# phandasm/waveform

Measured on NVIDIA H100. Metric: spectra/sec fused window+R2C-FFT+mag+smooth N=2048 batch=65536; %HBM roofline, higher is better.
Workload: dtype f32

## Files before the change

### waveform_b200/csrc/wf_engine.cu

```cuda
#include <cuda_runtime.h>

#include <cmath>
#include <cstdarg>
#include <algorithm>
#include <cstdio>
#include <cstdlib>
#include <cstring>
#include <new>
#include <string>
#include <vector>

#include "wf_kernels.cuh"
#include "wf_fast2048.cuh"
#include "wf_anyn.cuh"
#include "wf_wide.hpp"
#include "wf_v3.hpp"
#include "wf_team2048.hpp"
#include "wf_warp2.hpp"
#include "wf_par16384.hpp"
#include "wf_nvtx.hpp"
#include "wf_tables.hpp"
#include "wfstft.h"

using namespace wf;

struct wf_engine {
    Tables tab;
    int device = 0;
    int sm_count = 0;
    cudaStream_t stream = nullptr;
    cudaEvent_t ev0 = nullptr, ev1 = nullptr;
    bool ev_valid = false;
    std::string last_error;
    int64_t launches = 0;
    std::string last_kernel;
    bool hold_implicit = false;
    bool use_par16384 = true;
    bool use_warp2_display = true;
    bool use_warp2 = true;
    bool lazy_hold = true;
    bool split_runs = true;
    bool force_generic = false;
    int fast_maxw = 16;
    int fast_wpc_override = 0;
    bool use_pdl = true;
    int wide_r = 0;

    float *d_window = nullptr, *d_slope = nullptr, *d_rolloff = nullptr;
    float *d_tw = nullptr, *d_tw_post = nullptr;
    float *d_tw1 = nullptr, *d_tw2 = nullptr, *d_tw0 = nullptr;
    int fast_min_streams = 768;
    int team_w = 0;
    bool use_v3 = true;
    float *d_interp_idx = nullptr, *d_interp_w = nullptr, *d_gauss = nullptr;
    int *d_band_widths = nullptr, *d_band_offsets = nullptr;
    float *d_state = nullptr, *d_hold = nullptr;
    unsigned char *d_flags = nullptr;
    float *s_pcm = nullptr, *s_out_db = nullptr, *s_out_points = nullptr, *s_rms = nullptr, *s_peak = nullptr;
    unsigned char *s_skip = nullptr, *s_silent = nullptr;
    float *s_px = nullptr, *s_min = nullptr;
    float *s_gtab = nullptr;
    size_t s_gtab_cap = 0;
    std::vector<float> h_gtab;
    size_t s_px_cap = 0, s_min_cap = 0;
    float *s_scratch = nullptr;
    size_t s_scratch_cap = 0;
    size_t s_pcm_cap = 0, s_out_db_cap = 0, s_out_points_cap = 0, s_rms_cap = 0, s_peak_cap = 0, s_skip_cap = 0,
           s_silent_cap = 0;
    const void *zc_ptrs[9] = {};
    bool zc_ok = false, zc_dev = false, zc_valid = false;
    bool zero_copy = true;
    static constexpr int kMaxChunks = 16;
    cudaStream_t s_h2d = nullptr, s_d2h = nullptr;
    cudaEvent_t chunk_in[kMaxChunks] = {}, chunk_k[kMaxChunks] = {}, ev_fork = nullptr, ev_join = nullptr;
};

namespace {

thread_local std::string g_create_error;

int set_err(wf_engine *e, int code, const char *fmt, ...)
{
    if(e)
    {
        char buf[512];
        va_list ap;
        va_start(ap, fmt);
        vsnprintf(buf, sizeof(buf), fmt, ap);
        va_end(ap);
        e->last_error = buf;
    }
    return code;
}

#define WF_CUDA(e, call)                                                                                              \
    do                                                                                                                \
// ... 214 lines not shown
    stft_anyn_kernel<CC><<<grid, kAnyThreads, smem, st>>>(kp, plan);
    WF_CUDA(e, cudaGetLastError());
    e->launches++;
    e->last_kernel = "stft_anyn_kernel<" + std::to_string(CC) + "> N=" + std::to_string(e->tab.N);
    return WF_OK;
}

static void fast2048_geometry(int n_streams, int sm_count, int max_wpc, int *warps_per_cta, int *grid)
{
    *grid = std::min(n_streams, sm_count);
    const int per_cta = (n_streams + *grid - 1) / *grid;
    *warps_per_cta = std::max(std::min(8, max_wpc), std::min(max_wpc, per_cta));
}

template<int MAXW, bool TSM, bool GATE, bool EXTRA>
int launch_fast2048(wf_engine *e, const KParams &kp, cudaStream_t st)
{
    static thread_local bool configured[64] = {false};
    const int dev = e->device & 63;
    if(!configured[dev])
    {
        WF_CUDA(e, cudaFuncSetAttribute(stft2048_fast_kernel<MAXW, TSM, GATE, EXTRA>,
                                        cudaFuncAttributeMaxDynamicSharedMemorySize, fast::smem_bytes(MAXW)));
        configured[dev] = true;
    }
    int wpc = MAXW, grid = 1;
    fast2048_geometry(kp.n_streams, e->sm_count, MAXW, &wpc, &grid);
    if(e->fast_wpc_override > 0 && e->fast_wpc_override <= MAXW)
    {
        wpc = e->fast_wpc_override;
        grid = std::min(kp.n_streams, e->sm_count);
    }
    cudaLaunchConfig_t cfg{};
    cfg.gridDim = dim3((unsigned)grid);
    cfg.blockDim = dim3((unsigned)(wpc * 32));
    cfg.dynamicSmemBytes = fast::smem_bytes(wpc);
    cfg.stream = st;
    cudaLaunchAttribute attr[1];
    attr[0].id = cudaLaunchAttributeProgrammaticStreamSerialization;
    attr[0].val.programmaticStreamSerializationAllowed = e->use_pdl ? 1 : 0;
    cfg.attrs = attr;
    cfg.numAttrs = 1;
    WF_CUDA(e, cudaLaunchKernelEx(&cfg, stft2048_fast_kernel<MAXW, TSM, GATE, EXTRA>, kp));
    e->launches++;
    e->last_kernel = "stft2048_fast_kernel<" + std::to_string(MAXW) + "," + std::to_string((int)TSM) + "," + std::to_string((int)GATE) +
                     "," + std::to_string((int)EXTRA) + "> grid " + std::to_string(grid) + " x " + std::to_string(wpc) + " warps";
    return WF_OK;
}


int dispatch_fast2048(wf_engine *e, const KParams &kp, cudaStream_t st, bool extra)
{
    const bool tsm = kp.tsmooth != 0, gate = kp.gate != 0;
    const int maxw = e->fast_maxw;
#define WF_FAST_CASE(W, T, G, X)            \
    if(maxw == W && tsm == T && gate == G && extra == X) \
        return launch_fast2048<W, T, G, X>(e, kp, st);
    WF_FAST_CASE(16, true, true, false)
    WF_FAST_CASE(16, true, true, true)
    WF_FAST_CASE(16, true, false, false)
    WF_FAST_CASE(16, true, false, true)
    WF_FAST_CASE(16, false, true, false)
    WF_FAST_CASE(16, false, true, true)
    WF_FAST_CASE(16, false, false, false)
    WF_FAST_CASE(16, false, false, true)
    WF_FAST_CASE(12, true, true, false)
    WF_FAST_CASE(12, true, true, true)
    WF_FAST_CASE(12, true, false, false)
    WF_FAST_CASE(12, true, false, true)
    WF_FAST_CASE(12, false, true, false)
    WF_FAST_CASE(12, false, true, true)
    WF_FAST_CASE(12, false, false, false)
    WF_FAST_CASE(12, false, false, true)
#undef WF_FAST_CASE
    return set_err(e, WF_ERR_INVALID_ARG, "fast2048 dispatch fell through");
}

int fill_device(wf_engine *e, float *p, long long n, float v, cudaStream_t st)
{
    if(n <= 0)
        return WF_OK;
    int blocks = (int)std::min<long long>((n + 255) / 256, 1184);
    fill_kernel<<<blocks, 256, 0, st>>>(p, n, v);
    WF_CUDA(e, cudaGetLastError());
    e->launches++;
    return WF_OK;
}

int materialize_hold(wf_engine *e, cudaStream_t st)
{
    if(!e->hold_implicit)
        return WF_OK;
    const Tables &t = e->tab;
    const int S = t.cfg.max_streams;
    materialize_hold_kernel<<<std::min(S, e->sm_count * 8), 256, 0, st>>>(e->d_state, e->d_hold, e->d_flags, S, t.B,
                                                                          t.output_channels, t.db_min);
    WF_CUDA(e, cudaGetLastError());
    e->launches++;
    e->hold_implicit = false;
    return WF_OK;
}

int init_state(wf_engine *e, int first, int count, cudaStream_t st)
{
    const Tables &t = e->tab;
    const int cc = t.cfg.capture_channels, och = t.output_channels, B = t.B;
    WF_CUDA(e, cudaMemsetAsync(e->d_state + (size_t)first * cc * B, 0, (size_t)count * cc * B * sizeof(float), st));
    int rc = fill_device(e, e->d_hold + (size_t)first * och * B, (long long)count * och * B, t.db_min, st);
    if(rc)
        return rc;
    const bool below = !(t.db_min > (float)(t.cfg.floor_db - 10));
    WF_CUDA(e, cudaMemsetAsync(e->d_flags + first, below ? 6 : 0, (size_t)count, st));
    return WF_OK;
}

}

extern "C" {

int wf_abi_version(void) { return WF_ABI_VERSION; }

const char *wf_strerror(int status)
{
    switch(status)
    {
    case WF_OK: return "ok";
// ... 45 lines not shown
    c->interp_mode = WF_INTERP_CATROM;
    c->filter_mode = WF_FILTER_NONE;
    c->filter_radius = 1.5f;
    c->height = 225;
    c->channel_spacing = 0;
    c->rounded_caps = 0;
    c->min_bar_height = 0;
}

int wf_create(const wf_config *cfg, wf_engine **out)
{
    if(!cfg || !out)
        return WF_ERR_INVALID_ARG;
    *out = nullptr;
    if(cfg->struct_size != sizeof(wf_config))
        return WF_ERR_ABI;
    wf_engine *e = new(std::nothrow) wf_engine();
    if(!e)
        return WF_ERR_OOM;
    auto bail = [&](int code) {
        g_create_error = e->last_error;
        wf_destroy(e);
        return code;
    };

    const char *why = nullptr;
    int rc = build_tables(*cfg, e->tab, &why);
    if(rc != WF_OK)
    {
        set_err(e, rc, "%s", why ? why : "bad config");
        return bail(rc);
    }
    if(!supported_fft_size(e->tab.N))
        return bail(set_err(e, WF_ERR_UNSUPPORTED_FFT_SIZE, "fft_size %d unsupported", e->tab.N));

    int ndev = 0;
    if(cudaGetDeviceCount(&ndev) != cudaSuccess || ndev == 0)
    {
        cudaGetLastError();
        return bail(set_err(e, WF_ERR_NO_DEVICE, "no CUDA device"));
    }
    int dev = cfg->device;
    if(dev < 0)
    {
        if(cudaGetDevice(&dev) != cudaSuccess)
            return bail(set_err(e, WF_ERR_CUDA, "cudaGetDevice failed"));
    }
    if(dev >= ndev)
        return bail(set_err(e, WF_ERR_INVALID_ARG, "device %d out of range (%d devices)", dev, ndev));
    e->device = dev;
    {
        const char *fg = getenv("WF_FORCE_GENERIC");
        e->force_generic = fg && fg[0] == '1';
        const char *mw = getenv("WF_FAST_MAXW");
        if(mw && (atoi(mw) == 12 || atoi(mw) == 16))
            e->fast_maxw = atoi(mw);
        const char *np = getenv("WF_NO_PDL");
        e->use_pdl = !(np && np[0] == '1');
        const char *wr = getenv("WF_WIDE_R");
        if(wr)
            e->wide_r = atoi(wr);
        const char *fms = getenv("WF_FAST_MIN_STREAMS");
        if(fms)
            e->fast_min_streams = atoi(fms);
        const char *v3 = getenv("WF_V3");
        e->use_v3 = !(v3 && v3[0] == '0');
        const char *tw = getenv("WF_TEAM_W");
        if(tw)
            e->team_w = atoi(tw);
        const char *zc = getenv("WF_ZERO_COPY");
        e->zero_copy = !(zc && zc[0] == '0');
        const char *p16 = getenv("WF_PAR16384");
        e->use_par16384 = !(p16 && p16[0] == '0');
        const char *w2 = getenv("WF_WARP2");
        e->use_warp2 = !(w2 && w2[0] == '0');
        const char *w2d = getenv("WF_WARP2_DISPLAY");
        e->use_warp2_display = !(w2d && w2d[0] == '0');
        const char *lh = getenv("WF_LAZY_HOLD");
        e->lazy_hold = !(lh && lh[0] == '0');
        const char *sp = getenv("WF_SPLIT");
        e->split_runs = !(sp && sp[0] == '0');
        const char *wo = getenv("WF_FAST_WPC");
        if(wo)
            e->fast_wpc_override = atoi(wo);
    }

#define WF_TRY(x)                 \
    do                            \
    {                             \
        int _rc = (x);            \
        if(_rc != WF_OK)          \
            return bail(_rc);     \
    } while(0)
#define WF_CUDA_C(call)                                                                                      \
    do                                                                                                       \
    {                                                                                                        \
        cudaError_t _err = (call);                                                                           \
        if(_err != cudaSuccess)                                                                              \
            return bail(set_err(e, (_err == cudaErrorMemoryAllocation) ? WF_ERR_OOM : WF_ERR_CUDA, "%s: %s", \
                                #call, cudaGetErrorString(_err)));                                           \
    } while(0)

    WF_CUDA_C(cudaSetDevice(dev));
    cudaDeviceProp prop{};
    WF_CUDA_C(cudaGetDeviceProperties(&prop, dev));
    e->sm_count = prop.multiProcessorCount;
    if(prop.major != 9 || prop.minor != 0)
        return bail(set_err(e, WF_ERR_NO_DEVICE, "device %d is sm_%d%d; this library is built for sm_90a only", dev,
                            prop.major, prop.minor));
// ... 191 lines not shown
    kp.fast_peaks = t.cfg.fast_peaks;
    kp.stereo = t.cfg.stereo;
    kp.och = och;
    kp.dch = dch;
    kp.gate = t.cfg.silence_gate;
    kp.floor_m10 = (float)(t.cfg.floor_db - 10);
    kp.db_min = t.db_min;
    kp.normalize = t.cfg.normalize_volume;
    kp.vol_target = t.cfg.volume_target;
    kp.max_gain = t.cfg.max_gain;
    kp.write_hold = 1;
    kp.interp_idx = e->d_interp_idx;
    kp.interp_w = e->d_interp_w;
    kp.band_widths = e->d_band_widths;
    kp.band_offsets = e->d_band_offsets;
    kp.n_points = t.num_points;
    kp.n_sample = (t.cfg.display_mode == WF_DISPLAY_BAR && t.cfg.interp_mode != WF_INTERP_POINT) ? (int)t.interp_indices.size() : 0;
    kp.scratch_q = t.num_points + (dch * kp.n_sample + 3) / 4;
    kp.taps = t.interp_taps;
    kp.radius = t.interp_radius;
    kp.display_bar = (t.cfg.display_mode == WF_DISPLAY_BAR);
    kp.interp_mode = t.cfg.interp_mode;
    kp.gauss_w = e->d_gauss;
    kp.gauss_radius = t.gauss_radius;
    kp.gauss_size = (int)t.gauss.size();
    kp.gauss_sum = t.gauss_sum;
    kp.filter = (t.cfg.filter_mode == WF_FILTER_GAUSS);
    kp.out_pixels = b->out_pixels ? px_dev + (size_t)s0 * T * dch * t.num_points : nullptr;
    kp.out_min = b->out_min ? min_dev + (size_t)s0 * T * 2 : nullptr;
    kp.px_lo = t.px_lo;
    kp.px_hi = t.px_hi;
    kp.px_cpos = t.px_cpos;
    kp.ceiling_f = (float)t.cfg.ceiling_db;
    kp.dbrange_f = (float)(t.cfg.ceiling_db - t.cfg.floor_db);
    kp.mirror = t.cfg.mirror_freq_axis;

    size_t extra = 0;
    if(kp.out_points || kp.out_pixels || kp.out_min)
    {
        int groups = 1;
        switch(N)
        {
        case 128: groups = Geo<128>::GROUPS; break;
        case 256: groups = Geo<256>::GROUPS; break;
        case 512: groups = Geo<512>::GROUPS; break;
        case 1024: groups = Geo<1024>::GROUPS; break;
        case 2048: groups = Geo<2048>::GROUPS; break;
        default: groups = 1; break;
        }
        extra = (size_t)groups * 4 * (size_t)kp.scratch_q * sizeof(float);
    }
    const bool aligned16 = (((uintptr_t)kp.pcm & 15u) == 0) && ((b->stream_stride & 3) == 0) && ((b->hop & 3) == 0);
    const bool fast_ok = (N == 2048) && (cc == 1) && !t.cfg.stereo && kp.out_db && !kp.out_points && !kp.out_pixels &&
                         !kp.out_min && aligned16 && !e->force_generic;
    if(fast_ok)
    {
        const bool x = kp.slope || kp.rolloff || kp.normalize || kp.fast_peaks || kp.skip_mask || kp.out_peak || kp.g_tab;
        kp.lazy_hold = e->lazy_hold ? 1 : 0;
        kp.split = e->split_runs ? 1 : 0;
        if(kp.lazy_hold)
            e->hold_implicit = true;
        int W = 1;
        if(e->team_w != 1)
        {
            const int per_sm = (kp.n_streams + e->sm_count - 1) / e->sm_count;
            if(per_sm <= 8)
                W = (per_sm <= 1) ? 16 : (per_sm == 2) ? 8 : 4;
            if(e->team_w == 4 || e->team_w == 8 || e->team_w == 16)
                W = e->team_w;
            while(W > 1 && W > kp.n_frames)
                W /= 2;
            if(W == 2)
                W = 1;
        }
        if(W > 1)
        {
            const int tpc = 16 / W;
            const int grid = std::min(e->sm_count, kp.n_streams);
            WF_CUDA(e, team2048_launch(W, x, kp, grid, st, e->use_pdl, e->device));
            e->launches++;
            e->last_kernel = "stft2048_team_kernel<" + std::to_string(W) + "," + std::to_string((int)x) + "> grid " + std::to_string(grid) +
                             " x " + std::to_string(tpc) + " teams";
            return WF_OK;
        }
        return dispatch_fast2048(e, kp, st, x);
    }
    {
        const int rc = materialize_hold(e, st);
        if(rc)
            return rc;
    }
    const bool par_ok = (N == 16384) && e->use_par16384 && e->use_v3 && e->d_tw0 && (cc == 1) && !t.cfg.stereo && kp.out_db &&
                        !kp.out_points && !kp.out_pixels && !kp.out_min && !e->force_generic;
    if(par_ok)
    {
        const bool x = kp.slope || kp.rolloff || kp.normalize || kp.fast_peaks || kp.skip_mask || kp.out_peak || kp.g_tab;
        WF_CUDA(e, par16384_launch(x, kp, e->d_tw1, e->d_tw2, e->d_tw0, st, e->device));
        e->launches++;
        e->last_kernel = "stft16384_parity_kernel<" + std::to_string((int)x) + "> " + std::to_string(kp.n_streams) + " clusters of 2";
        return WF_OK;
    }
    const bool disp = kp.out_points || kp.out_pixels || kp.out_min;
    const bool warp2_ok = e->use_warp2 && (cc == 1) && !t.cfg.stereo && aligned16 &&
                          (disp ? (e->use_warp2_display && !e->force_generic && (warp2_supported(N) || warp2_pow2_supported(N)))
                                : (warp2_supported(N) && kp.out_db));
    if(warp2_ok)
    {
// ... 444 lines not shown
```

### waveform_b200/csrc/wf_fast2048.cuh

```cuda
#pragma once
#include "wf_kernels.cuh"

namespace wf {

namespace fast {

constexpr int kN = 2048;
constexpr int kM = 1024;
constexpr int kWarpBufBytes = 32 * 33 * 8;
constexpr int kStateBytes = 16 * 32 * 8;
constexpr int kWarpBytes = kWarpBufBytes + kStateBytes + 16;
constexpr int kTableBytes = (1024 + 1024 + 512) * 8;
constexpr int kMaxWarpsPerCta = 16;
constexpr int smem_bytes(int warps_per_cta) { return kTableBytes + warps_per_cta * kWarpBytes; }

__device__ __forceinline__ uint32_t smem_u32(const void *p) { return (uint32_t)__cvta_generic_to_shared(p); }

__device__ __forceinline__ void mbar_init(uint64_t *bar, uint32_t count)
{
    asm volatile("mbarrier.init.shared::cta.b64 [%0], %1;" ::"r"(smem_u32(bar)), "r"(count) : "memory");
}
__device__ __forceinline__ void mbar_expect_tx(uint64_t *bar, uint32_t bytes)
{
    asm volatile("mbarrier.arrive.expect_tx.shared::cta.b64 _, [%0], %1;" ::"r"(smem_u32(bar)), "r"(bytes) : "memory");
}
__device__ __forceinline__ void mbar_wait(uint64_t *bar, uint32_t parity)
{
    asm volatile(
        "{\n\t"
        ".reg .pred p;\n\t"
        "WAIT_LOOP:\n\t"
        "mbarrier.try_wait.parity.shared::cta.b64 p, [%0], %1;\n\t"
        "@p bra DONE;\n\t"
        "bra WAIT_LOOP;\n\t"
        "DONE:\n\t"
        "}" ::"r"(smem_u32(bar)),
        "r"(parity)
        : "memory");
}
__device__ __forceinline__ void tma_load_1d(void *dst_smem, const void *src_gmem, uint32_t bytes, uint64_t *bar)
{
    asm volatile("cp.async.bulk.shared::cluster.global.mbarrier::complete_tx::bytes [%0], [%1], %2, [%3];" ::"r"(
                     smem_u32(dst_smem)),
                 "l"(src_gmem), "r"(bytes), "r"(smem_u32(bar))
                 : "memory");
}
__device__ __forceinline__ void fence_proxy_async()
{
    asm volatile("fence.proxy.async.shared::cta;" ::: "memory");
}
__device__ __forceinline__ float sqrt_approx(float x)
{
    float r;
    asm("sqrt.approx.ftz.f32 %0, %1;" : "=f"(r) : "f"(x));
    return r;
}

__device__ __forceinline__ float lg2_approx_ftz(float x)
{
    float r;
    asm("lg2.approx.ftz.f32 %0, %1;" : "=f"(r) : "f"(x));
    return r;
}
__device__ __forceinline__ pk::c64 dbfs2(float m1, float m2, float db_min)
{
    constexpr float k = 6.02059991327962390f;
    pk::c64 d = pk::mul(pk::make(lg2_approx_ftz(m1), lg2_approx_ftz(m2)), pk::make(k, k));
    float d1, d2;
    pk::split(d, d1, d2);
    return pk::make(fmaxf(d1, db_min), fmaxf(d2, db_min));
}

}

template<int MAXW, bool TSM, bool GATE, bool EXTRA>
__global__ void __launch_bounds__(MAXW * 32, 1) stft2048_fast_kernel(const __grid_constant__ KParams p)
{
    using namespace fast;
    extern __shared__ __align__(128) unsigned char smem_raw[];
    float2 *s_win = reinterpret_cast<float2 *>(smem_raw);
    float2 *s_twA = s_win + 1024;
    float2 *s_twP = s_twA + 1024;
    const int warp = threadIdx.x >> 5;
    const int lane = threadIdx.x & 31;
    const int warps_per_cta = blockDim.x >> 5;
    unsigned char *wbase = reinterpret_cast<unsigned char *>(s_twP + 512) + warp * kWarpBytes;
    float2 *buf = reinterpret_cast<float2 *>(wbase);
    float2 *sst = reinterpret_cast<float2 *>(wbase + kWarpBufBytes) + lane;
    uint64_t *mbar = reinterpret_cast<uint64_t *>(wbase + kWarpBufBytes + kStateBytes);

    for(int i = threadIdx.x; i < 1024; i += blockDim.x)
    {
        {
            const float2 w = (p.window2 != nullptr) ? __ldg(p.window2 + i) : make_float2(1.0f, 1.0f);
            s_win[i] = make_float2(w.x * p.coef_half, w.y * p.coef_half);
        }
        s_twA[i] = __ldg(p.tw + (((i >> 5) * (i & 31)) & 1023));
        if(i < 512)
            s_twP[i] = __ldg(p.tw_post + i);
    }
    int *seg_done = reinterpret_cast<int *>(mbar + 1);
    if(lane == 0)
    {
        mbar_init(mbar, 1);
        *seg_done = 0;
        asm volatile("fence.mbarrier_init.release.cluster;" ::: "memory");
    }
    __syncthreads();
    asm volatile("griddepcontrol.launch_dependents;" ::: "memory");
    asm volatile("griddepcontrol.wait;" ::: "memory");

    const int S = p.n_streams, T = p.n_frames;
    const int G = gridDim.x;
    const int n_local = (S > (int)blockIdx.x) ? (S - (int)blockIdx.x + G - 1) / G : 0;
    constexpr int B = kM;
    uint32_t phase = 0;

    const int jp = (32 - lane) & 31;
    const int kb = jp + (lane == 0 ? 32 : 0);
    const int k2_q0 = (lane == 0) ? 512 : (kb + 992);

    const int rounds_whole = (n_local + warps_per_cta - 1) / warps_per_cta;
    const bool split = (p.split != 0) && (n_local >= warps_per_cta) && (T > 1) &&
                       (2 * (rounds_whole * warps_per_cta - n_local) * T > 3 * warps_per_cta);
    int u0 = 0, u1 = 0;
    if(split)
    {
        const int U = n_local * T, per = (U + warps_per_cta - 1) / warps_per_cta;
        u0 = min(warp * per, U);
        u1 = min(u0 + per, U);
    }
    const int full0 = (u0 + T - 1) / T, full1 = u1 / T;
    const int has_head = (split && (u1 % T) != 0) ? 1 : 0, has_tail = (split && (u0 % T) != 0) ? 1 : 0;
    const int nseg = split ? (has_head + max(full1 - full0, 0) + has_tail)
                           : ((n_local > warp) ? (n_local - warp + warps_per_cta - 1) / warps_per_cta : 0);
    auto segment = [&](int j, int &li, int &t0, int &t1) {
        if(!split)
        {
            li = warp + j * warps_per_cta;
            t0 = 0;
            t1 = T;
            return;
        }
        if(has_head && j == 0)
        {
            li = full1;
            t0 = 0;
            t1 = u1 % T;
            return;
        }
        j -= has_head;
        if(j < full1 - full0)
        {
            li = full0 + j;
            t0 = 0;
            t1 = T;
            return;
        }
        li = u0 / T;
        t0 = u0 % T;
        t1 = T;
    };

    if(nseg > 0 && lane == 0)
    {
        int li, t0, t1;
        segment(0, li, t0, t1);
        mbar_expect_tx(mbar, kN * 4);
        tma_load_1d(buf, p.pcm + (size_t)(blockIdx.x + li * G) * p.stream_stride + (size_t)t0 * p.hop, kN * 4, mbar);
    }

    for(int j = 0; j < nseg; ++j)
    {
        int li, t0, t1;
        segment(j, li, t0, t1);
        const int s = (int)blockIdx.x + li * G;
        int s_next = -1, t0_next = 0;
        if(j + 1 < nseg)
        {
            int li2, t12;
            segment(j + 1, li2, t0_next, t12);
            s_next = (int)blockIdx.x + li2 * G;
        }
        if(t0 > 0)
        {
            int *prev_done = reinterpret_cast<int *>(wbase - kWarpBytes + kWarpBufBytes + kStateBytes + 8);
            if(lane == 0)
                while(atomicAdd(prev_done, 0) == 0)
                    ;
            __syncwarp();
            __threadfence_block();
        }
        {
            const float *sp = p.state + (size_t)s * B;
#pragma unroll
            for(int q = 0; q < 16; ++q)
                sst[q * 32] = make_float2(sp[lane + 32 * q], sp[(q == 0) ? k2_q0 : (kb + 32 * (31 - q))]);
        }
        const unsigned char fl = p.flags[s];
        bool last_silent = (fl & 1u) != 0;
        bool prev_out_silent = (fl & 2u) != 0;
        const bool hold_lazy = (fl & 8u) != 0;
        bool last_from_state = false;
        const float *pcm_s = p.pcm + (size_t)s * p.stream_stride;
        float *hold_s = p.hold_db + (size_t)s * B;

#pragma unroll 1
        for(int t = t0; t < t1; ++t)
        {
            mbar_wait(mbar, phase);
            phase ^= 1u;
            pk::c64 v[32];
            unsigned long long nzbits = 0;
            const pk::c64 *buf64 = reinterpret_cast<const pk::c64 *>(buf);
            const pk::c64 *win64 = reinterpret_cast<const pk::c64 *>(s_win);
#pragma unroll
            for(int pidx = 0; pidx < 32; ++pidx)
            {
                v[pidx] = buf64[lane + 32 * pidx];
                nzbits |= v[pidx];
            }
#pragma unroll
            for(int pidx = 0; pidx < 32; ++pidx)
                v[pidx] = pk::mul(v[pidx], win64[lane + 32 * pidx]);
            const bool nz = __any_sync(0xffffffffu, (nzbits & 0x7fffffff7fffffffull) != 0ull);

#pragma unroll
            for(int pass = 0; pass < 2; ++pass)
            {
                pk::dft_bitrev<32>(v);
                if(pass == 0)
                {
                    __syncwarp();
#pragma unroll
                    for(int k2 = 0; k2 < 32; ++k2)
                    {
                        pk::c64 a = v[bitrev<32>(k2)];
                        if(k2 > 0)
                            a = pk::cmul(a, reinterpret_cast<const pk::c64 *>(s_twA)[k2 * 32 + lane]);
                        reinterpret_cast<pk::c64 *>(buf)[lane * 33 + k2] = a;
                    }
                    __syncwarp();
#pragma unroll
                    for(int n1 = 0; n1 < 32; ++n1)
                        v[n1] = buf64[n1 * 33 + lane];
                    __syncwarp();
                    if(t + 1 == t1 && s_next >= 0 && t0_next == 0)
                        asm volatile("prefetch.global.L2 [%0];" ::"l"(p.state + (size_t)s_next * B + lane * 32));
                    if(lane == 0)
                    {
                        const float *next = nullptr;
                        if(t + 1 < t1)
                            next = pcm_s + (size_t)(t + 1) * p.hop;
                        else if(s_next >= 0)
                            next = p.pcm + (size_t)s_next * p.stream_stride + (size_t)t0_next * p.hop;
                        if(next != nullptr)
                        {
                            fence_proxy_async();
                            mbar_expect_tx(mbar, kN * 4);
                            tma_load_1d(buf, next, kN * 4, mbar);
                        }
                    }
                }
            }

            const bool skip_all = EXTRA && (p.skip_mask != nullptr) && (p.skip_mask[(size_t)s * T + t] != 0);
            bool do_proc = !skip_all;
            if(!skip_all)
            {
                if(nz)
                    last_silent = false;
                else if(GATE)
                {
                    if(last_silent)
                        do_proc = false;
                    else if(prev_out_silent)
                    {
                        last_silent = true;
                        do_proc = false;
                    }
                }
            }

            float *odb = p.out_db + ((size_t)s * T + t) * B;
            float vc = 0.0f;
            if(EXTRA && p.normalize)
            {
                const float rms = (p.input_rms != nullptr) ? p.input_rms[(size_t)s * T + t] : 0.0f;
                vc = fminf(p.vol_target - dbfs(rms, p.db_min), p.max_gain);
            }
            bool outs = true;
            float peak = -INFINITY;
            const float2 gt = (EXTRA && p.g_tab != nullptr) ? __ldg(p.g_tab + t) : make_float2(p.g, p.g2);

            if(do_proc && !last_silent)
            {
#pragma unroll
                for(int q = 0; q < 16; ++q)
                {
                    const int k1 = lane + 32 * q;
                    const int k2 = (q == 0) ? k2_q0 : (kb + 32 * (31 - q));
                    const pk::c64 a = v[bitrev<32>(q)];
                    unsigned long long bp = __shfl_sync(0xffffffffu, v[bitrev<32>(31 - q)], jp);
                    if(lane == 0)
                        bp = v[bitrev<32>((32 - q) & 31)];
                    const pk::c64 b = pk::conj(bp);
                    const pk::c64 sum = pk::add(a, b);
                    const pk::c64 o = pk::mul_neg_i(pk::sub(a, b));
                    const pk::c64 wo = pk::cmul(o, reinterpret_cast<const pk::c64 *>(s_twP)[q * 32 + lane]);
                    const pk::c64 y1 = pk::add(sum, wo);
                    const pk::c64 y2 = pk::sub(sum, wo);
                    const pk::c64 s1 = pk::mul(y1, y1), s2 = pk::mul(y2, y2);
                    float p1 = pk::re(s1) + pk::im(s1);
                    float p2 = pk::re(s2) + pk::im(s2);
                    if(q == 0)
                    {
                        const pk::c64 x512 = v[bitrev<32>(16)];
                        const pk::c64 sq = pk::mul(x512, x512);
                        const float p512 = 4.0f * (pk::re(sq) + pk::im(sq));
                        p2 = (lane == 0) ? p512 : p2;
                    }
                    pk::c64 m = pk::make(sqrt_approx(p1), sqrt_approx(p2));
                    if(EXTRA && p.slope != nullptr)
                        m = pk::mul(m, pk::make(__ldg(p.slope + k1), __ldg(p.slope + k2)));
                    pk::c64 *sst64 = reinterpret_cast<pk::c64 *>(sst);
                    if(TSM)
                    {
                        pk::c64 old = sst64[q * 32];
                        if(EXTRA && p.fast_peaks)
                            old = pk::make(fmaxf(pk::re(m), pk::re(old)), fmaxf(pk::im(m), pk::im(old)));
                        m = pk::fma(pk::make(gt.x, gt.x), old, pk::mul(pk::make(gt.y, gt.y), m));
                    }
                    sst64[q * 32] = m;
                    float d1, d2;
                    pk::split(dbfs2(pk::re(m), pk::im(m), p.db_min), d1, d2);
                    if(EXTRA)
                    {
                        if(p.normalize)
                        {
                            if(k1 >= 1)
                                d1 += vc;
                            d2 += vc;
                        }
                        if(p.rolloff != nullptr)
                        {
                            if(k1 >= 1)
                                d1 = fmaxf(d1 - __ldg(p.rolloff + k1), p.db_min);
                            d2 = fmaxf(d2 - __ldg(p.rolloff + k2), p.db_min);
                        }
                        if(k1 >= 1)
                            peak = fmaxf(peak, d1);
                        peak = fmaxf(peak, d2);
                    }
                    if(GATE)
                        outs &= !(d1 > p.floor_m10) & !(d2 > p.floor_m10);
                    stg_stream(odb + k1, d1);
                    stg_stream(odb + k2, d2);
                }
                last_from_state = true;
            }
            else
            {
                const float *prev_db = (t > 0) ? (odb - B) : hold_s;
                const bool from_state = (t == 0) && hold_lazy;
#pragma unroll 1
                for(int q = 0; q < 16; ++q)
                {
                    const int k1 = lane + 32 * q;
                    const int k2 = (q == 0) ? k2_q0 : (kb + 32 * (31 - q));
                    float o1, o2;
                    if(from_state)
                    {
                        const float2 stv = sst[q * 32];
                        pk::split(dbfs2(stv.x, stv.y, p.db_min), o1, o2);
                    }
                    else
                    {
                        o1 = prev_db[k1];
                        o2 = prev_db[k2];
                    }
                    if(!last_silent)
                    {
                        o1 = dbfs(o1, p.db_min);
                        o2 = dbfs(o2, p.db_min);
                        if(EXTRA)
                        {
                            if(p.normalize)
                            {
                                if(k1 >= 1)
                                    o1 += vc;
                                o2 += vc;
                            }
                            if(p.rolloff != nullptr)
                            {
                                if(k1 >= 1)
                                    o1 = fmaxf(o1 - __ldg(p.rolloff + k1), p.db_min);
                                o2 = fmaxf(o2 - __ldg(p.rolloff + k2), p.db_min);
                            }
                        }
                    }
                    outs &= !(o1 > p.floor_m10) & !(o2 > p.floor_m10);
                    if(k1 >= 1)
                        peak = fmaxf(peak, o1);
                    peak = fmaxf(peak, o2);
                    odb[k1] = o1;
                    odb[k2] = o2;
                }
                last_from_state = false;
            }
            if(GATE && !last_silent)
                prev_out_silent = __all_sync(0xffffffffu, outs);
            if(p.out_silent != nullptr && lane == 0)
                p.out_silent[(size_t)s * T + t] = last_silent ? 1 : 0;
            if(EXTRA)
            {
                if(p.out_peak != nullptr)
                {
                    const float gm = group_max<32>(peak, nullptr);
                    if(lane == 0)
                        atomic_max_float(p.out_peak + t, gm);
                }
            }
        }

        {
            float *sp = p.state + (size_t)s * B;
            const float *last = p.out_db + ((size_t)s * T + (t1 - 1)) * B;
            const bool plain = !EXTRA || (!p.normalize && p.rolloff == nullptr);
            const bool lazy = last_from_state && plain && (p.lazy_hold != 0);
#pragma unroll
            for(int q = 0; q < 16; ++q)
            {
                const int k1 = lane + 32 * q;
                const int k2 = (q == 0) ? k2_q0 : (kb + 32 * (31 - q));
                const float2 stv = sst[q * 32];
                sp[k1] = stv.x;
                sp[k2] = stv.y;
                if(p.write_hold && !lazy)
                {
                    if(last_from_state && plain)
                    {
                        float h1, h2;
                        pk::split(dbfs2(stv.x, stv.y, p.db_min), h1, h2);
                        hold_s[k1] = h1;
                        hold_s[k2] = h2;
                    }
                    else
                    {
                        hold_s[k1] = last[k1];
                        hold_s[k2] = last[k2];
                    }
                }
            }
            if(lane == 0)
                p.flags[s] = (unsigned char)((last_silent ? 1u : 0u) | (prev_out_silent ? 2u : 0u) | 4u | (lazy ? 8u : 0u));
        }
        if(t1 < T)
        {
            __threadfence_block();
            __syncwarp();
            if(lane == 0)
                atomicExch(seg_done, 1);
        }
        __syncwarp();
    }
}

}
```

### waveform_b200/csrc/wf_team2048.cuh

```cuda
#pragma once
#include "wf_fast2048.cuh"

namespace wf {

namespace team {
constexpr int kCtlBytes = 64;
constexpr int kWarps = 16;
constexpr int smem_bytes() { return fast::kTableBytes + kWarps * fast::kWarpBytes + kWarps * kCtlBytes; }

__device__ __forceinline__ void bar_sync(int id, int nthreads)
{
    asm volatile("bar.sync %0, %1;" ::"r"(id), "r"(nthreads) : "memory");
}
}

template<int W, bool EXTRA>
__global__ void __launch_bounds__(team::kWarps * 32, 1) stft2048_team_kernel(const __grid_constant__ KParams p)
{
    using namespace fast;
    constexpr int TPC = team::kWarps / W;
    constexpr int BW = kM / W;
    constexpr int BPL = BW / 32;
    constexpr int VEC = (BPL >= 4) ? 4 : 2;
    constexpr int B = kM;
    extern __shared__ __align__(128) unsigned char smem_raw[];
    float2 *s_win = reinterpret_cast<float2 *>(smem_raw);
    float2 *s_twA = s_win + 1024;
    float2 *s_twP = s_twA + 1024;
    const int warp = threadIdx.x >> 5;
    const int lane = threadIdx.x & 31;
    const int tm = warp / W;
    const int wi = warp % W;
    unsigned char *warps_base = reinterpret_cast<unsigned char *>(s_twP + 512);
    unsigned char *wbase = warps_base + warp * kWarpBytes;
    float2 *buf = reinterpret_cast<float2 *>(wbase);
    float *mymag = reinterpret_cast<float *>(wbase + kWarpBufBytes);
    uint64_t *mbar = reinterpret_cast<uint64_t *>(wbase + kWarpBufBytes + kStateBytes);
    unsigned char *ctl = warps_base + team::kWarps * kWarpBytes + tm * team::kCtlBytes;
    volatile unsigned char *ctl_nz = ctl;
    volatile unsigned char *ctl_outs = ctl + 16;
    const int bar_id = 1 + tm;

    for(int i = threadIdx.x; i < 1024; i += blockDim.x)
    {
        const float2 w = (p.window2 != nullptr) ? __ldg(p.window2 + i) : make_float2(1.0f, 1.0f);
        s_win[i] = make_float2(w.x * p.coef_half, w.y * p.coef_half);
        s_twA[i] = __ldg(p.tw + (((i >> 5) * (i & 31)) & 1023));
        if(i < 512)
            s_twP[i] = __ldg(p.tw_post + i);
    }
    if(lane == 0)
    {
        mbar_init(mbar, 1);
        asm volatile("fence.mbarrier_init.release.cluster;" ::: "memory");
    }
    __syncthreads();
    asm volatile("griddepcontrol.launch_dependents;" ::: "memory");
    asm volatile("griddepcontrol.wait;" ::: "memory");

    const int S = p.n_streams, T = p.n_frames;
    const int G = gridDim.x;
    const int n_local = (S > (int)blockIdx.x) ? (S - (int)blockIdx.x + G - 1) / G : 0;
    uint32_t phase = 0;
    const bool tsm = p.tsmooth != 0, gate = p.gate != 0;

    const int jp = (32 - lane) & 31;
    const int kb = jp + (lane == 0 ? 32 : 0);
    const int k2_q0 = (lane == 0) ? 512 : (kb + 992);
    const int b0 = wi * BW + lane * BPL;

    if(tm < n_local && wi < T && lane == 0)
    {
        mbar_expect_tx(mbar, kN * 4);
        tma_load_1d(buf, p.pcm + (size_t)(blockIdx.x + tm * G) * p.stream_stride + (size_t)wi * p.hop, kN * 4, mbar);
    }

    for(int li = tm; li < n_local; li += TPC)
    {
        const int s = (int)blockIdx.x + li * G;
        const bool have_next_stream = (li + TPC) < n_local;
        const float *pcm_s = p.pcm + (size_t)s * p.stream_stride;
        float *hold_s = p.hold_db + (size_t)s * B;
        float *state_s = p.state + (size_t)s * B;

        float st[BPL];
#pragma unroll
        for(int j = 0; j < BPL; j += VEC)
        {
            if constexpr(VEC == 4)
            {
                const float4 x = *reinterpret_cast<const float4 *>(state_s + b0 + j);
// ... 86 lines not shown
                    const int k1 = lane + 32 * q;
                    const int k2 = (q == 0) ? k2_q0 : (kb + 32 * (31 - q));
                    const pk::c64 a = v[bitrev<32>(q)];
                    unsigned long long bp = __shfl_sync(0xffffffffu, v[bitrev<32>(31 - q)], jp);
                    if(lane == 0)
                        bp = v[bitrev<32>((32 - q) & 31)];
                    const pk::c64 b = pk::conj(bp);
                    const pk::c64 sum = pk::add(a, b);
                    const pk::c64 o = pk::mul_neg_i(pk::sub(a, b));
                    const pk::c64 wo = pk::cmul(o, reinterpret_cast<const pk::c64 *>(s_twP)[q * 32 + lane]);
                    const pk::c64 y1 = pk::add(sum, wo);
                    const pk::c64 y2 = pk::sub(sum, wo);
                    const pk::c64 s1 = pk::mul(y1, y1), s2 = pk::mul(y2, y2);
                    float p1 = pk::re(s1) + pk::im(s1);
                    float p2 = pk::re(s2) + pk::im(s2);
                    if(q == 0)
                    {
                        const pk::c64 x512 = v[bitrev<32>(16)];
                        const pk::c64 sq = pk::mul(x512, x512);
                        const float p512 = 4.0f * (pk::re(sq) + pk::im(sq));
                        p2 = (lane == 0) ? p512 : p2;
                    }
                    float m1 = sqrt_approx(p1), m2 = sqrt_approx(p2);
                    if(EXTRA && p.slope != nullptr)
                    {
                        m1 *= __ldg(p.slope + k1);
                        m2 *= __ldg(p.slope + k2);
                    }
                    mymag[k1] = m1;
                    mymag[k2] = m2;
                }
                if(lane == 0)
                    ctl_nz[wi] = nz ? 1 : 0;
            }
            team::bar_sync(bar_id, W * 32);

            bool round_done = false;
            if(t0 + W <= T && !(EXTRA && p.skip_mask != nullptr))
            {
                bool all_nz = true;
#pragma unroll
                for(int i = 0; i < W; ++i)
                    all_nz &= ctl_nz[i] != 0;
                if(all_nz)
                {
                    last_silent = false;
                    float *odb0 = p.out_db + ((size_t)s * T + t0) * B + b0;
                    float dl[BPL];
#pragma unroll
                    for(int i = 0; i < W; ++i)
                    {
                        const int tt = t0 + i;
                        const float2 gt = (EXTRA && p.g_tab != nullptr) ? __ldg(p.g_tab + tt) : make_float2(p.g, p.g2);
                        const float *mg = reinterpret_cast<const float *>(warps_base + (size_t)(tm * W + i) * kWarpBytes + kWarpBufBytes) + b0;
                        float d[BPL];
#pragma unroll
                        for(int j = 0; j < BPL; j += VEC)
                        {
                            float m[4];
                            if constexpr(VEC == 4)
                            {
                                const float4 x = *reinterpret_cast<const float4 *>(mg + j);
                                m[0] = x.x, m[1] = x.y, m[2] = x.z, m[3] = x.w;
                            }
                            else
                            {
                                const float2 x = *reinterpret_cast<const float2 *>(mg + j);
                                m[0] = x.x, m[1] = x.y;
                            }
#pragma unroll
                            for(int u = 0; u < VEC; ++u)
                            {
                                float mm = m[u];
                                if(tsm)
                                {
                                    float old = st[j + u];
                                    if(EXTRA && p.fast_peaks)
                                        old = fmaxf(mm, old);
                                    mm = fmaf(gt.x, old, gt.y * mm);
                                }
                                st[j + u] = mm;
                            }
                        }
#pragma unroll
                        for(int j = 0; j < BPL; j += 2)
                            pk::split(dbfs2(st[j], st[j + 1], p.db_min), d[j], d[j + 1]);
                        if(EXTRA)
                        {
                            float vc = 0.0f;
                            if(p.normalize)
                            {
                                const float rms = (p.input_rms != nullptr) ? p.input_rms[(size_t)s * T + tt] : 0.0f;
                                vc = fminf(p.vol_target - dbfs(rms, p.db_min), p.max_gain);
                            }
                            float peak = -INFINITY;
#pragma unroll
                            for(int j = 0; j < BPL; ++j)
                            {
                                const int k = b0 + j;
                                if(k >= 1)
                                {
                                    if(p.normalize)
                                        d[j] += vc;
                                    if(p.rolloff != nullptr)
                                        d[j] = fmaxf(d[j] - __ldg(p.rolloff + k), p.db_min);
                                    peak = fmaxf(peak, d[j]);
                                }
// ... 31 lines not shown
                            outs &= !(dl[j] > p.floor_m10);
                        outs_lane = outs;
                        pos_valid = false;
                    }
                    if(p.out_silent != nullptr && wi == 0 && lane < W)
                        p.out_silent[(size_t)s * T + t0 + lane] = 0;
                    last_from_state = true;
                    round_done = true;
                }
            }
#pragma unroll 1
            for(int i = 0; i < W && !round_done; ++i)
            {
                const int tt = t0 + i;
                if(tt >= T)
                    break;
                const bool nz = ctl_nz[i] != 0;
                const bool skip_all = EXTRA && (p.skip_mask != nullptr) && (p.skip_mask[(size_t)s * T + tt] != 0);
                bool do_proc = !skip_all;
                if(!skip_all)
                {
                    if(nz)
                        last_silent = false;
                    else if(gate)
                    {
                        if(last_silent)
                            do_proc = false;
                        else
                        {
                            if(!pos_valid)
                            {
                                pos = team_all(outs_lane);
                                pos_valid = true;
                            }
                            if(pos)
                            {
                                last_silent = true;
                                do_proc = false;
                            }
                        }
                    }
                }
                const float2 gt = (EXTRA && p.g_tab != nullptr) ? __ldg(p.g_tab + tt) : make_float2(p.g, p.g2);
                float *odb = p.out_db + ((size_t)s * T + tt) * B + b0;
                float vc = 0.0f;
                if(EXTRA && p.normalize)
                {
                    const float rms = (p.input_rms != nullptr) ? p.input_rms[(size_t)s * T + tt] : 0.0f;
                    vc = fminf(p.vol_target - dbfs(rms, p.db_min), p.max_gain);
                }
                float d[BPL];
                if(do_proc && !last_silent)
                {
                    const float *mg = reinterpret_cast<const float *>(warps_base + (size_t)(tm * W + i) * kWarpBytes + kWarpBufBytes) + b0;
#pragma unroll
                    for(int j = 0; j < BPL; j += VEC)
                    {
                        float m[4];
                        if constexpr(VEC == 4)
                        {
                            const float4 x = *reinterpret_cast<const float4 *>(mg + j);
                            m[0] = x.x, m[1] = x.y, m[2] = x.z, m[3] = x.w;
                        }
                        else
                        {
                            const float2 x = *reinterpret_cast<const float2 *>(mg + j);
                            m[0] = x.x, m[1] = x.y;
                        }
#pragma unroll
                        for(int u = 0; u < VEC; ++u)
                        {
                            float mm = m[u];
                            if(tsm)
                            {
                                float old = st[j + u];
                                if(EXTRA && p.fast_peaks)
                                    old = fmaxf(mm, old);
                                mm = fmaf(gt.x, old, gt.y * mm);
                            }
                            st[j + u] = mm;
                        }
                    }
#pragma unroll
                    for(int j = 0; j < BPL; j += 2)
                    {
                        pk::split(dbfs2(st[j], st[j + 1], p.db_min), d[j], d[j + 1]);
                    }
                    if(EXTRA)
                    {
#pragma unroll
                        for(int j = 0; j < BPL; ++j)
                        {
                            const int k = b0 + j;
                            if(k >= 1)
                            {
                                if(p.normalize)
                                    d[j] += vc;
                                if(p.rolloff != nullptr)
                                    d[j] = fmaxf(d[j] - __ldg(p.rolloff + k), p.db_min);
                            }
                        }
                    }
                    last_from_state = true;
                }
                else
                {
                    const bool from_state = (tt == 0) && hold_lazy;
// ... 106 lines not shown
```

Measured before the change: 192.9 million.

## Add TMA landing buffer, register smoothing state, and bulk async row stores

Each warp gets a separate landing buffer for the input frame, so the next frame's TMA load can be issued right after the current frame is read instead of after the first FFT pass. Smoothing state moves from shared memory into registers. Output dB rows are staged in shared memory and written with cp.async.bulk stores instead of per-lane streaming stores. The larger per-warp shared footprint lowers the maximum warps per CTA from 16 to 12, which cuts parallelism per SM, and the fast path now also requires a 16-byte-aligned output pointer.

```diff
diff --git a/waveform_b200/csrc/wf_engine.cu b/waveform_b200/csrc/wf_engine.cu
--- a/waveform_b200/csrc/wf_engine.cu
+++ b/waveform_b200/csrc/wf_engine.cu
@@ -41,7 +41,6 @@
     bool lazy_hold = true;
     bool split_runs = true;
     bool force_generic = false;
-    int fast_maxw = 16;
     int fast_wpc_override = 0;
     bool use_pdl = true;
     int wide_r = 0;
@@ -362,26 +361,17 @@
 int dispatch_fast2048(wf_engine *e, const KParams &kp, cudaStream_t st, bool extra)
 {
     const bool tsm = kp.tsmooth != 0, gate = kp.gate != 0;
-    const int maxw = e->fast_maxw;
-#define WF_FAST_CASE(W, T, G, X)            \
-    if(maxw == W && tsm == T && gate == G && extra == X) \
-        return launch_fast2048<W, T, G, X>(e, kp, st);
-    WF_FAST_CASE(16, true, true, false)
-    WF_FAST_CASE(16, true, true, true)
-    WF_FAST_CASE(16, true, false, false)
-    WF_FAST_CASE(16, true, false, true)
-    WF_FAST_CASE(16, false, true, false)
-    WF_FAST_CASE(16, false, true, true)
-    WF_FAST_CASE(16, false, false, false)
-    WF_FAST_CASE(16, false, false, true)
-    WF_FAST_CASE(12, true, true, false)
-    WF_FAST_CASE(12, true, true, true)
-    WF_FAST_CASE(12, true, false, false)
-    WF_FAST_CASE(12, true, false, true)
-    WF_FAST_CASE(12, false, true, false)
-    WF_FAST_CASE(12, false, true, true)
-    WF_FAST_CASE(12, false, false, false)
-    WF_FAST_CASE(12, false, false, true)
+#define WF_FAST_CASE(T, G, X)                  \
+    if(tsm == T && gate == G && extra == X) \
+        return launch_fast2048<fast::kMaxWarpsPerCta, T, G, X>(e, kp, st);
+    WF_FAST_CASE(true, true, false)
+    WF_FAST_CASE(true, true, true)
+    WF_FAST_CASE(true, false, false)
+    WF_FAST_CASE(true, false, true)
+    WF_FAST_CASE(false, true, false)
+    WF_FAST_CASE(false, true, true)
+    WF_FAST_CASE(false, false, false)
+    WF_FAST_CASE(false, false, true)
 #undef WF_FAST_CASE
     return set_err(e, WF_ERR_INVALID_ARG, "fast2048 dispatch fell through");
 }
@@ -533,9 +523,6 @@
     {
         const char *fg = getenv("WF_FORCE_GENERIC");
         e->force_generic = fg && fg[0] == '1';
-        const char *mw = getenv("WF_FAST_MAXW");
-        if(mw && (atoi(mw) == 12 || atoi(mw) == 16))
-            e->fast_maxw = atoi(mw);
         const char *np = getenv("WF_NO_PDL");
         e->use_pdl = !(np && np[0] == '1');
         const char *wr = getenv("WF_WIDE_R");
@@ -833,7 +820,7 @@
     }
     const bool aligned16 = (((uintptr_t)kp.pcm & 15u) == 0) && ((b->stream_stride & 3) == 0) && ((b->hop & 3) == 0);
     const bool fast_ok = (N == 2048) && (cc == 1) && !t.cfg.stereo && kp.out_db && !kp.out_points && !kp.out_pixels &&
-                         !kp.out_min && aligned16 && !e->force_generic;
+                         !kp.out_min && aligned16 && (((uintptr_t)kp.out_db & 15u) == 0) && !e->force_generic;
     if(fast_ok)
     {
         const bool x = kp.slope || kp.rolloff || kp.normalize || kp.fast_peaks || kp.skip_mask || kp.out_peak || kp.g_tab;
diff --git a/waveform_b200/csrc/wf_fast2048.cuh b/waveform_b200/csrc/wf_fast2048.cuh
--- a/waveform_b200/csrc/wf_fast2048.cuh
+++ b/waveform_b200/csrc/wf_fast2048.cuh
@@ -7,12 +7,13 @@
 
 constexpr int kN = 2048;
 constexpr int kM = 1024;
-constexpr int kWarpBufBytes = 32 * 33 * 8;
-constexpr int kStateBytes = 16 * 32 * 8;
-constexpr int kWarpBytes = kWarpBufBytes + kStateBytes + 16;
+constexpr int kLandBytes = kN * 4;
+constexpr int kXposeBytes = 32 * 33 * 8;
+constexpr int kWarpBytes = kLandBytes + kXposeBytes + 16;
 constexpr int kTableBytes = (1024 + 1024 + 512) * 8;
-constexpr int kMaxWarpsPerCta = 16;
+constexpr int kMaxWarpsPerCta = 12;
 constexpr int smem_bytes(int warps_per_cta) { return kTableBytes + warps_per_cta * kWarpBytes; }
+static_assert(smem_bytes(kMaxWarpsPerCta) <= 227 * 1024, "one CTA per SM must fit");
 
 __device__ __forceinline__ uint32_t smem_u32(const void *p) { return (uint32_t)__cvta_generic_to_shared(p); }
 
@@ -49,6 +50,21 @@
 {
     asm volatile("fence.proxy.async.shared::cta;" ::: "memory");
 }
+__device__ __forceinline__ void bulk_store_1d(void *dst_gmem, const void *src_smem, uint32_t bytes)
+{
+    asm volatile("cp.async.bulk.global.shared::cta.bulk_group [%0], [%1], %2;" ::"l"(dst_gmem), "r"(smem_u32(src_smem)), "r"(bytes)
+                 : "memory");
+    asm volatile("cp.async.bulk.commit_group;" ::: "memory");
+}
+__device__ __forceinline__ void bulk_wait_read()
+{
+    asm volatile("cp.async.bulk.wait_group.read 0;" ::: "memory");
+}
+__device__ __forceinline__ void bulk_wait_written()
+{
+    asm volatile("cp.async.bulk.wait_group 0;" ::: "memory");
+    asm volatile("fence.proxy.async.global;" ::: "memory");
+}
 __device__ __forceinline__ float sqrt_approx(float x)
 {
     float r;
@@ -77,6 +93,7 @@
 __global__ void __launch_bounds__(MAXW * 32, 1) stft2048_fast_kernel(const __grid_constant__ KParams p)
 {
     using namespace fast;
+    static_assert(MAXW <= kMaxWarpsPerCta, "shared memory holds at most kMaxWarpsPerCta warps");
     extern __shared__ __align__(128) unsigned char smem_raw[];
     float2 *s_win = reinterpret_cast<float2 *>(smem_raw);
     float2 *s_twA = s_win + 1024;
@@ -85,9 +102,11 @@
     const int lane = threadIdx.x & 31;
     const int warps_per_cta = blockDim.x >> 5;
     unsigned char *wbase = reinterpret_cast<unsigned char *>(s_twP + 512) + warp * kWarpBytes;
-    float2 *buf = reinterpret_cast<float2 *>(wbase);
-    float2 *sst = reinterpret_cast<float2 *>(wbase + kWarpBufBytes) + lane;
-    uint64_t *mbar = reinterpret_cast<uint64_t *>(wbase + kWarpBufBytes + kStateBytes);
+    float2 *land = reinterpret_cast<float2 *>(wbase);
+    float2 *buf = reinterpret_cast<float2 *>(wbase + kLandBytes);
+    float *row = reinterpret_cast<float *>(buf);
+    uint64_t *mbar = reinterpret_cast<uint64_t *>(wbase + kWarpBytes - 16);
+    pk::c64 st[16];
 
     for(int i = threadIdx.x; i < 1024; i += blockDim.x)
     {
@@ -167,7 +186,7 @@
         int li, t0, t1;
         segment(0, li, t0, t1);
         mbar_expect_tx(mbar, kN * 4);
-        tma_load_1d(buf, p.pcm + (size_t)(blockIdx.x + li * G) * p.stream_stride + (size_t)t0 * p.hop, kN * 4, mbar);
+        tma_load_1d(land, p.pcm + (size_t)(blockIdx.x + li * G) * p.stream_stride + (size_t)t0 * p.hop, kN * 4, mbar);
     }
 
     for(int j = 0; j < nseg; ++j)
@@ -184,7 +203,7 @@
         }
         if(t0 > 0)
         {
-            int *prev_done = reinterpret_cast<int *>(wbase - kWarpBytes + kWarpBufBytes + kStateBytes + 8);
+            int *prev_done = reinterpret_cast<int *>(reinterpret_cast<unsigned char *>(seg_done) - kWarpBytes);
             if(lane == 0)
                 while(atomicAdd(prev_done, 0) == 0)
                     ;
@@ -195,7 +214,7 @@
             const float *sp = p.state + (size_t)s * B;
 #pragma unroll
             for(int q = 0; q < 16; ++q)
-                sst[q * 32] = make_float2(sp[lane + 32 * q], sp[(q == 0) ? k2_q0 : (kb + 32 * (31 - q))]);
+                st[q] = pk::make(sp[lane + 32 * q], sp[(q == 0) ? k2_q0 : (kb + 32 * (31 - q))]);
         }
         const unsigned char fl = p.flags[s];
         bool last_silent = (fl & 1u) != 0;
@@ -212,13 +231,29 @@
             phase ^= 1u;
             pk::c64 v[32];
             unsigned long long nzbits = 0;
+            const pk::c64 *land64 = reinterpret_cast<const pk::c64 *>(land);
             const pk::c64 *buf64 = reinterpret_cast<const pk::c64 *>(buf);
             const pk::c64 *win64 = reinterpret_cast<const pk::c64 *>(s_win);
 #pragma unroll
             for(int pidx = 0; pidx < 32; ++pidx)
             {
-                v[pidx] = buf64[lane + 32 * pidx];
+                v[pidx] = land64[lane + 32 * pidx];
                 nzbits |= v[pidx];
+            }
+            __syncwarp();
+            if(lane == 0)
+            {
+                const float *next = nullptr;
+                if(t + 1 < t1)
+                    next = pcm_s + (size_t)(t + 1) * p.hop;
+                else if(s_next >= 0)
+                    next = p.pcm + (size_t)s_next * p.stream_stride + (size_t)t0_next * p.hop;
+                if(next != nullptr)
+                {
+                    fence_proxy_async();
+                    mbar_expect_tx(mbar, kN * 4);
+                    tma_load_1d(land, next, kN * 4, mbar);
+                }
             }
 #pragma unroll
             for(int pidx = 0; pidx < 32; ++pidx)
@@ -231,6 +266,8 @@
                 pk::dft_bitrev<32>(v);
                 if(pass == 0)
                 {
+                    if(lane == 0)
+                        bulk_wait_read();
                     __syncwarp();
 #pragma unroll
                     for(int k2 = 0; k2 < 32; ++k2)
@@ -247,20 +284,6 @@
                     __syncwarp();
                     if(t + 1 == t1 && s_next >= 0 && t0_next == 0)
                         asm volatile("prefetch.global.L2 [%0];" ::"l"(p.state + (size_t)s_next * B + lane * 32));
-                    if(lane == 0)
-                    {
-                        const float *next = nullptr;
-                        if(t + 1 < t1)
-                            next = pcm_s + (size_t)(t + 1) * p.hop;
-                        else if(s_next >= 0)
-                            next = p.pcm + (size_t)s_next * p.stream_stride + (size_t)t0_next * p.hop;
-                        if(next != nullptr)
-                        {
-                            fence_proxy_async();
-                            mbar_expect_tx(mbar, kN * 4);
-                            tma_load_1d(buf, next, kN * 4, mbar);
-                        }
-                    }
                 }
             }
 
@@ -323,15 +346,14 @@
                     pk::c64 m = pk::make(sqrt_approx(p1), sqrt_approx(p2));
                     if(EXTRA && p.slope != nullptr)
                         m = pk::mul(m, pk::make(__ldg(p.slope + k1), __ldg(p.slope + k2)));
-                    pk::c64 *sst64 = reinterpret_cast<pk::c64 *>(sst);
                     if(TSM)
                     {
-                        pk::c64 old = sst64[q * 32];
+                        pk::c64 old = st[q];
                         if(EXTRA && p.fast_peaks)
                             old = pk::make(fmaxf(pk::re(m), pk::re(old)), fmaxf(pk::im(m), pk::im(old)));
                         m = pk::fma(pk::make(gt.x, gt.x), old, pk::mul(pk::make(gt.y, gt.y), m));
                     }
-                    sst64[q * 32] = m;
+                    st[q] = m;
                     float d1, d2;
                     pk::split(dbfs2(pk::re(m), pk::im(m), p.db_min), d1, d2);
                     if(EXTRA)
@@ -354,8 +376,8 @@
                     }
                     if(GATE)
                         outs &= !(d1 > p.floor_m10) & !(d2 > p.floor_m10);
-                    stg_stream(odb + k1, d1);
-                    stg_stream(odb + k2, d2);
+                    row[k1] = d1;
+                    row[k2] = d2;
                 }
                 last_from_state = true;
             }
@@ -363,7 +385,13 @@
             {
                 const float *prev_db = (t > 0) ? (odb - B) : hold_s;
                 const bool from_state = (t == 0) && hold_lazy;
-#pragma unroll 1
+                if(t > 0)
+                {
+                    if(lane == 0)
+                        bulk_wait_written();
+                    __syncwarp();
+                }
+#pragma unroll
                 for(int q = 0; q < 16; ++q)
                 {
                     const int k1 = lane + 32 * q;
@@ -371,8 +399,9 @@
                     float o1, o2;
                     if(from_state)
                     {
-                        const float2 stv = sst[q * 32];
-                        pk::split(dbfs2(stv.x, stv.y, p.db_min), o1, o2);
+                        float s1, s2;
+                        pk::split(st[q], s1, s2);
+                        pk::split(dbfs2(s1, s2, p.db_min), o1, o2);
                     }
                     else
                     {
@@ -403,11 +432,15 @@
                     if(k1 >= 1)
                         peak = fmaxf(peak, o1);
                     peak = fmaxf(peak, o2);
-                    odb[k1] = o1;
-                    odb[k2] = o2;
+                    row[k1] = o1;
+                    row[k2] = o2;
                 }
                 last_from_state = false;
             }
+            fence_proxy_async();
+            __syncwarp();
+            if(lane == 0)
+                bulk_store_1d(odb, row, B * 4);
             if(GATE && !last_silent)
                 prev_out_silent = __all_sync(0xffffffffu, outs);
             if(p.out_silent != nullptr && lane == 0)
@@ -425,7 +458,6 @@
 
         {
             float *sp = p.state + (size_t)s * B;
-            const float *last = p.out_db + ((size_t)s * T + (t1 - 1)) * B;
             const bool plain = !EXTRA || (!p.normalize && p.rolloff == nullptr);
             const bool lazy = last_from_state && plain && (p.lazy_hold != 0);
 #pragma unroll
@@ -433,7 +465,8 @@
             {
                 const int k1 = lane + 32 * q;
                 const int k2 = (q == 0) ? k2_q0 : (kb + 32 * (31 - q));
-                const float2 stv = sst[q * 32];
+                float2 stv;
+                pk::split(st[q], stv.x, stv.y);
                 sp[k1] = stv.x;
                 sp[k2] = stv.y;
                 if(p.write_hold && !lazy)
@@ -447,8 +480,8 @@
                     }
                     else
                     {
-                        hold_s[k1] = last[k1];
-                        hold_s[k2] = last[k2];
+                        hold_s[k1] = row[k1];
+                        hold_s[k2] = row[k2];
                     }
                 }
             }
@@ -457,6 +490,8 @@
         }
         if(t1 < T)
         {
+            if(lane == 0)
+                bulk_wait_written();
             __threadfence_block();
             __syncwarp();
             if(lane == 0)
@@ -464,6 +499,8 @@
         }
         __syncwarp();
     }
-}
-
-}
+    if(lane == 0)
+        bulk_wait_written();
+}
+
+}
diff --git a/waveform_b200/csrc/wf_team2048.cuh b/waveform_b200/csrc/wf_team2048.cuh
--- a/waveform_b200/csrc/wf_team2048.cuh
+++ b/waveform_b200/csrc/wf_team2048.cuh
@@ -6,7 +6,10 @@
 namespace team {
 constexpr int kCtlBytes = 64;
 constexpr int kWarps = 16;
-constexpr int smem_bytes() { return fast::kTableBytes + kWarps * fast::kWarpBytes + kWarps * kCtlBytes; }
+constexpr int kWarpBufBytes = 32 * 33 * 8;
+constexpr int kMagBytes = 1024 * 4;
+constexpr int kWarpBytes = kWarpBufBytes + kMagBytes + 16;
+constexpr int smem_bytes() { return fast::kTableBytes + kWarps * kWarpBytes + kWarps * kCtlBytes; }
 
 __device__ __forceinline__ void bar_sync(int id, int nthreads)
 {
@@ -32,11 +35,11 @@
     const int tm = warp / W;
     const int wi = warp % W;
     unsigned char *warps_base = reinterpret_cast<unsigned char *>(s_twP + 512);
-    unsigned char *wbase = warps_base + warp * kWarpBytes;
+    unsigned char *wbase = warps_base + warp * team::kWarpBytes;
     float2 *buf = reinterpret_cast<float2 *>(wbase);
-    float *mymag = reinterpret_cast<float *>(wbase + kWarpBufBytes);
-    uint64_t *mbar = reinterpret_cast<uint64_t *>(wbase + kWarpBufBytes + kStateBytes);
-    unsigned char *ctl = warps_base + team::kWarps * kWarpBytes + tm * team::kCtlBytes;
+    float *mymag = reinterpret_cast<float *>(wbase + team::kWarpBufBytes);
+    uint64_t *mbar = reinterpret_cast<uint64_t *>(wbase + team::kWarpBufBytes + team::kMagBytes);
+    unsigned char *ctl = warps_base + team::kWarps * team::kWarpBytes + tm * team::kCtlBytes;
     volatile unsigned char *ctl_nz = ctl;
     volatile unsigned char *ctl_outs = ctl + 16;
     const int bar_id = 1 + tm;
@@ -229,7 +232,7 @@
                     {
                         const int tt = t0 + i;
                         const float2 gt = (EXTRA && p.g_tab != nullptr) ? __ldg(p.g_tab + tt) : make_float2(p.g, p.g2);
-                        const float *mg = reinterpret_cast<const float *>(warps_base + (size_t)(tm * W + i) * kWarpBytes + kWarpBufBytes) + b0;
+                        const float *mg = reinterpret_cast<const float *>(warps_base + (size_t)(tm * W + i) * team::kWarpBytes + team::kWarpBufBytes) + b0;
                         float d[BPL];
 #pragma unroll
                         for(int j = 0; j < BPL; j += VEC)
@@ -367,7 +370,7 @@
                 float d[BPL];
                 if(do_proc && !last_silent)
                 {
-                    const float *mg = reinterpret_cast<const float *>(warps_base + (size_t)(tm * W + i) * kWarpBytes + kWarpBufBytes) + b0;
+                    const float *mg = reinterpret_cast<const float *>(warps_base + (size_t)(tm * W + i) * team::kWarpBytes + team::kWarpBufBytes) + b0;
 #pragma unroll
                     for(int j = 0; j < BPL; j += VEC)
                     {
```

New measurement: 207.0 million (median of 6 runs). 1.07x the previous value.
